# szpiech/garlic

Measured on AMD Instinct MI355X. Metric: LOD-windows/sec (SNPs x inds / winsize), higher is better.
Workload: dtype f64

## Files before the change

garlic_amd/csrc/garlic_hip.hip:

```cpp
#include "../../include/garlic_hip.h"
#include "lod_kernels.hpp"
#include "variant_kernels.hpp"
#include "ld_kernels.hpp"
#include "ld_multi_kernel.hpp"
#include "tgls_ring_kernel.hpp"
#include "tgls_feed_kernel.hpp"
#include "tgls_feed_multi_kernel.hpp"
#include "wlod_strip_kernel.hpp"
#include "wlod_small_kernel.hpp"
#include "coverage_kernel.hpp"
#include "roh_segments_kernel.hpp"
#include "feed_kernel.hpp"
#include "wlod_feed_kernel.hpp"
#include "feed_sort_kernel.hpp"

#include <algorithm>
#include <chrono>
#include <functional>
#include <memory>
#include <mutex>
#include <queue>
#include <cmath>
#include <cstdarg>
#include <cstdio>
// ... 166 lines not shown

struct garlic_panel {
    garlic_ctx *ctx = nullptr;
    int32_t nchr = 0;
    int32_t nind = 0;
    int64_t nloci = 0;
    int64_t nind_pad = 0;
    int64_t nwordrows = 0;
    std::vector<int32_t> chr_nloci;
    std::vector<int64_t> chr_off;
    std::vector<int32_t> pos, cs, ce;
    std::vector<double> gpos, freq;
    bool have_map = false, have_freq = false, have_geno = false, have_gpos = false;
    DevBuf<uint32_t> d_packed;
    DevBuf<int32_t> d_pos, d_cs, d_ce;
    DevBuf<int64_t> d_chr_off;
    DevBuf<double> d_tab;
    bool tab_valid = false;
    double tab_error = 0;
    double tab_min = 0, tabgl_min = 0, glterms_min = 0;
    bool tab_all_finite = false;
    bool seg_valid = false;
    int32_t seg_max_gap = 0;
    std::vector<int64_t> boundaries;
    DevBuf<int32_t> d_blk_counts, d_blk_offsets, d_total;
    DevBuf<int64_t> d_boundaries;
    DevBuf<ChainItem> d_items;
    DevBuf<FeedItem> d_feed_items;
    DevBuf<FillItem> d_fill;
    DevBuf<int32_t> d_counter;
    DevBuf<ChrDev> d_chrs;
    DevBuf<int16_t> d_stage16;
    DevBuf<int64_t> d_row_counts;
    bool have_gl = false;
    std::vector<double> gl_values;
    std::unordered_map<uint64_t, int> gl_code;
    DevBuf<uint8_t> d_codes;
    DevBuf<double> d_tabgl;
    bool tabgl_valid = false;
    DevBuf<double> d_glterms;
    bool glterms_valid = false, glterms_scaled = false;
    int32_t glterms_M = 0;
    double glterms_mu = 0.0;
    int64_t terms_budget = 0;
    DevBuf<double> d_slab[2];
    hipStream_t slab_stream = nullptr;
    hipEvent_t ev_slab_begin = nullptr, ev_slab_built[2] = {}, ev_slab_read[2] = {};
    DevBuf<int32_t> d_slab_queues;
    int32_t last_slab_blocks = 0, last_n_slabs = 0;

    int tabgl_ncodes = 0;
    bool gl_cont = false;
    DevBuf<double> d_glval;
    bool gl_vals_dropped = false;
    bool gl_cover_required = false;
    std::vector<uint8_t> gl_cover;
    DevBuf<double> d_freq;
    bool dfreq_valid = false;
    int gl_terms_by = 0;
    bool have_ld = false, wlod_use_gl = false, rld_valid = false;
    int32_t last_chain_kind = 0;
    int32_t last_feed_form = GARLIC_FEED_FROM_SCORES;
    int64_t last_feed_doubles = 0;
    int32_t ld_winsize = 0;
    struct LdSet {
        int32_t W = 0, group = -1;
        DevBuf<double> skew;
    };
    std::vector<std::unique_ptr<LdSet>> ld_sets;
    int32_t ld_group = -1;
    bool ld_multi_active = false;
    int32_t ld_pair_passes = 0, ld_sum_passes = 0;
    DevBuf<double> d_rld, d_decay, d_stage64;
    DevBuf<uint64_t> d_phase;
    uint64_t geno_epoch = 0;
    CovBits cov_pending{nullptr, nullptr, 0.0};
    bool cov_written = false;
    bool have_phase = false;
    struct {
        DevBuf<uint64_t> sub, m, h, o;
        DevBuf<int32_t> loc, pair, loc_planes;
        DevBuf<double> hf, fwd, bwd, ld;
        DevBuf<LdSumChr> sum_chrs;
        DevBuf<LdPairChr> pair_chrs;
        DevBuf<LdMultiChr> multi_chrs;
        uint64_t planes_key = 0;
        bool planes_valid = false;
        bool fuse_request = false, fused_done = false;
        void release()
        {
            sub.release(); m.release(); h.release(); o.release(); loc.release(); pair.release(); loc_planes.release();
            hf.release(); fwd.release(); bwd.release(); ld.release(); sum_chrs.release(); pair_chrs.release();
            multi_chrs.release();
            planes_valid = false;
        }
    } lds;
    DevBuf<double> d_skew, d_wtab;
    DevBuf<uint8_t> d_valid;
    DevBuf<int2> d_tiles, d_segs;
    DevBuf<WlodStrip> d_strips;
    DevBuf<int32_t> d_feed_blocks;
    std::vector<double> h_tab, h_decay;
    bool wtab_valid = false;
    double wtab_error = 0.0, wtab_mu = 0.0;
    int32_t wtab_M = 0;
    int64_t wtab_rows = 0;
    bool decay_valid = false;
    int32_t decay_M = 0;
    double decay_mu = 0;
    struct ScoreBuf {
        double *p = nullptr;
        size_t cap = 0;
        garlic_ctx *ctx = nullptr;
        int reserve(garlic_ctx *c, size_t n)
        {
            if (n <= cap) return GARLIC_OK;
            release();
            void *q = nullptr;
            int rc = score_alloc(c, n * sizeof(double), &q);
            if (rc) return rc;
            p = (double *)q; cap = n; ctx = c;
            return GARLIC_OK;
        }
        void adopt(garlic_ctx *c, void *q, size_t n) { release(); p = (double *)q; cap = n; ctx = c; }
        void release()
        {
            if (p) (void)score_free(ctx, p);
            p = nullptr; cap = 0;
        }
    } d_out;
    bool placing = false;
    DevBuf<double> d_feed;
    int32_t feed_order = GARLIC_FEED_ORDER_REFERENCE;
    FeedSortScratch fs;
    struct FeedSlot {
        hipStream_t stream = nullptr;
        hipEvent_t ev0 = nullptr, ev1 = nullptr;
        DevBuf<FeedItem> items;
        DevBuf<ChrDev> chrs;
        DevBuf<int32_t> counter;
        DevBuf<int64_t> row_counts;
        DevBuf<double> out, feed;
        FeedSortScratch fs;
    };
    std::vector<FeedSlot *> feed_slots;
    DevBuf<ChainItem> d_multi_items;
    DevBuf<ChrDev> d_multi_chrs, d_multi_gchrs;
    DevBuf<int32_t> d_multi_queues;
    std::vector<int32_t> multi_forms, multi_groups;
    int32_t multi_chain_launches = 0, multi_term_builds = 0;
    garlic_call_stats stats{};
    bool stats_pending = false;
    int stats_slot = 0;
    int64_t n_count_timeouts = 0;
    struct Placement { int32_t drawn = 0, rounds = 0; float best_ms = 0, median_ms = 0, worst_ms = 0, target_ms = 0; int32_t reached = 0; };
    Placement placement;
    struct PlanKey {
        int mode = -1;
        int32_t W = 0, max_gap = 0, ind_begin = 0, ind_count = 0, pitch_align = 0, thin_step = 0;
        uint64_t blocks_hash = 0;
        bool wlod_tuned = false, wlod_strip = false, feed_kernel = false;
        int32_t slab_blocks = 0;
        auto tie() const { return std::tie(mode, W, max_gap, ind_begin, ind_count, pitch_align, thin_step, blocks_hash, wlod_tuned, wlod_strip, feed_kernel, slab_blocks); }
        bool operator==(const PlanKey &o) const { return tie() == o.tie(); }
    };
    struct Plan {
        bool valid = false;
        PlanKey key;
        size_t n_items = 0, n_fill = 0, n_feed_items = 0;
        int feed_per_cu = 1;
        int32_t n_tiles = 0, n_segs = 0, n_strips = 0, n_feed_blocks = 0;
        int64_t n_runs = 0, n_valid = 0;
        struct Slab { int32_t b0, b1; size_t item0, n_items; };
        std::vector<Slab> slabs;
    } plan;
// ... 2229 lines not shown
            if ((rc = p->lds.hf.reserve(p->nloci)) || (rc = p->lds.fwd.reserve(2 * n + 256))) return rc;
            hipLaunchKernelGGL(ld_homfreq_kernel, dim3((unsigned)((p->nloci + 255) / 256)), dim3(256), 0, s, p->lds.loc_planes.p, p->nloci,
                               p->lds.hf.p);
            a_hf = p->lds.hf.p;
            a_c = p->lds.fwd.p;
        }
        if (e == hipSuccess && lds > 48 * 1024) e = hipFuncSetAttribute(fn, hipFuncAttributeMaxDynamicSharedMemorySize, (int)lds);
        if (e != hipSuccess) return fail(GARLIC_ERR_HIP, "LD counts: %s", hipGetErrorString(e));
        const uint64_t *a_m = d_m.p, *a_h = d_h.p;
        const LdPairChr *a_pc = d_pc.p;
        int a_nblk = nblk, a_nchr = p->nchr, a_w = winsize;
        int64_t a_nloci = p->nloci;
        void *kargs[] = {(void *)&a_m, (void *)&a_h, (void *)&a_nblk, (void *)&a_nloci, (void *)&a_pc, (void *)&a_nchr, (void *)&a_w, (void *)&pair,
                         (void *)&a_hf, (void *)&a_c};
        e = hipLaunchKernel(fn, dim3((unsigned)blocks), dim3(256), kargs, lds, s);
        if (e == hipSuccess) e = hipStreamSynchronize(s);
        if (e != hipSuccess) return fail(GARLIC_ERR_HIP, "LD counts: %s", hipGetErrorString(e));
        p->lds.fused_done = fuse_hr2;
    }
    if (pair_lane) {
        std::vector<LdPairChr> pc;
        int64_t blocks = 0;
        for (int c = 0; c < p->nchr; c++) {
            pc.push_back(LdPairChr{p->chr_off[c], p->chr_off[c + 1], blocks});
            blocks += (p->chr_nloci[c] + LD_LANE_T - 1) / LD_LANE_T;
        }
        DevBuf<LdPairChr> &d_pc = p->lds.pair_chrs;
        if ((rc = d_pc.reserve(pc.size()))) return rc;
        e = hipMemcpyAsync(d_pc.p, pc.data(), sizeof(LdPairChr) * pc.size(), hipMemcpyHostToDevice, s);
        const void *fn = lane_dc == 16 ? (phased ? (const void *)ld_pair_lane_kernel<true, 16> : (const void *)ld_pair_lane_kernel<false, 16>)
                                       : (phased ? (const void *)ld_pair_lane_kernel<true, 32> : (const void *)ld_pair_lane_kernel<false, 32>);
        if (e == hipSuccess && lane_lds > 48 * 1024) e = hipFuncSetAttribute(fn, hipFuncAttributeMaxDynamicSharedMemorySize, (int)lane_lds);
        if (e != hipSuccess) return fail(GARLIC_ERR_HIP, "LD counts: %s", hipGetErrorString(e));
        const uint64_t *a_m = d_m.p, *a_h = d_h.p, *a_o = phased ? d_o.p : nullptr, *a_f = phased ? p->d_phase.p : nullptr;
        const LdPairChr *a_pc = d_pc.p;
        int a_nblk = nblk, a_nchr = p->nchr, a_w = winsize, a_stage = lane_stage;
        int64_t a_nloci = p->nloci;
        void *kargs[] = {(void *)&a_m, (void *)&a_h, (void *)&a_o, (void *)&a_f, (void *)&a_nblk, (void *)&a_nloci, (void *)&a_pc,
                         (void *)&a_nchr, (void *)&a_w, (void *)&a_stage, (void *)&pair};
        e = hipLaunchKernel(fn, dim3((unsigned)blocks), dim3(LD_LANE_T), kargs, lane_lds, s);
        if (e == hipSuccess) e = hipStreamSynchronize(s);
        if (e != hipSuccess) return fail(GARLIC_ERR_HIP, "LD counts: %s", hipGetErrorString(e));
    }
    if (pair_flat) {
        const unsigned grid = (unsigned)(((int64_t)p->nloci * winsize + 255) / 256);
        if (phased)
            hipLaunchKernelGGL(ld_pair_flat_kernel<true>, dim3(grid), dim3(256), 0, s, d_m.p, d_h.p, d_o.p, p->d_phase.p, nblk,
                               p->nloci, p->d_chr_off.p, p->nchr, winsize, pair);
        else
            hipLaunchKernelGGL(ld_pair_flat_kernel<false>, dim3(grid), dim3(256), 0, s, d_m.p, d_h.p, (const uint64_t *)nullptr,
                               (const uint64_t *)nullptr, nblk, p->nloci, p->d_chr_off.p, p->nchr, winsize, pair);
    }
    for (int c = 0; !pair_tiled && !pair_flat && !pair_lane && !pair_mfma && c < p->nchr; c++) {
        if (phased)
            hipLaunchKernelGGL(ld_pair_phased_kernel, dim3((unsigned)p->chr_nloci[c]), dim3(256), 0, s, d_m.p,
                               d_h.p, d_o.p, p->d_phase.p, nblk, p->nloci, p->chr_off[c], p->chr_off[c + 1],
                               winsize, pair);
        else
            hipLaunchKernelGGL(ld_pair_kernel, dim3((unsigned)p->chr_nloci[c]), dim3(256), 0, s, d_m.p, d_h.p,
                               nblk, p->nloci, p->chr_off[c], p->chr_off[c + 1], winsize, pair);
    }
    e = hipGetLastError();
    if (e == hipSuccess && where == GARLIC_HOST) {
        e = hipMemcpyAsync(locus_counts, loc, sizeof(int32_t) * p->nloci * 2, hipMemcpyDeviceToHost, s);
        if (e == hipSuccess)
            e = hipMemcpyAsync(pair_counts, pair, sizeof(int32_t) * npair, hipMemcpyDeviceToHost, s);
    }
    if (e == hipSuccess) e = hipStreamSynchronize(s);
    if (e != hipSuccess) return fail(GARLIC_ERR_HIP, "LD counts: %s", hipGetErrorString(e));
    return GARLIC_OK;
}

int garlic_ld_finish(garlic_panel *p, int32_t winsize, int32_t phased, const int32_t *locus_counts,
                     const int32_t *pair_counts, double *ld_out, int32_t where)
{
    int rc;
    if ((rc = ld_check(p, winsize, phased))) return rc;
    if (!locus_counts || !pair_counts) return fail(GARLIC_ERR_INVALID, "count buffers are required");
    hipStream_t s = p->ctx->stream;
    const size_t n = (size_t)p->nloci * winsize;
    DevBuf<int32_t> &d_loc = p->lds.loc, &d_pair = p->lds.pair;
    DevBuf<double> &d_hf = p->lds.hf, &d_fwd = p->lds.fwd, &d_bwd = p->lds.bwd, &d_ld = p->lds.ld;
    DevBuf<LdSumChr> &d_sum_chrs = p->lds.sum_chrs;
    const int32_t *loc = locus_counts, *pair = pair_counts;
    hipError_t e = hipSuccess;
    if (where == GARLIC_HOST) {
        if ((rc = d_loc.reserve((size_t)p->nloci * 2)) || (rc = d_pair.reserve(n * 2))) return rc;
        e = hipMemcpyAsync(d_loc.p, locus_counts, sizeof(int32_t) * p->nloci * 2, hipMemcpyHostToDevice, s);
        if (e == hipSuccess)
            e = hipMemcpyAsync(d_pair.p, pair_counts, sizeof(int32_t) * n * 2, hipMemcpyHostToDevice, s);
        loc = d_loc.p; pair = d_pair.p;
    }
    if (winsize <= LD_SMALL_MAX_W && !getenv("GARLIC_LD_NO_FLAT")) {
        if ((rc = d_hf.reserve(p->nloci))) return rc;
        double *ld = ld_out;
        if (where == GARLIC_HOST || !ld_out) {
            if ((rc = d_ld.reserve(n))) return rc;
            ld = d_ld.p;
        }
        if (e == hipSuccess) e = hipMemsetAsync(ld, 0, sizeof(double) * n, s);
        if (e == hipSuccess && phased) e = hipMemcpyAsync(d_hf.p, p->freq.data(), sizeof(double) * p->nloci, hipMemcpyHostToDevice, s);
        if (e != hipSuccess) return fail(GARLIC_ERR_HIP, "LD finish: %s", hipGetErrorString(e));
        if (!phased)
            hipLaunchKernelGGL(ld_homfreq_kernel, dim3((unsigned)((p->nloci + 255) / 256)), dim3(256), 0, s, loc, p->nloci, d_hf.p);
        garlic_ctx *ctx = p->ctx;
        const int slot = (int)(ctx->n_calls % garlic_ctx::HIST);
        (void)hipEventRecord(ctx->hist0[slot], s);
        hipLaunchKernelGGL(ld_sum_flat_kernel, dim3((unsigned)((n + 255) / 256)), dim3(256), 0, s, pair, d_hf.p, p->d_chr_off.p,
                           p->nchr, p->nloci, winsize, ld);
        (void)hipEventRecord(ctx->hist1[slot], s);
        ctx->n_calls++;
        e = hipGetLastError();
        if (e != hipSuccess) return fail(GARLIC_ERR_HIP, "LD finish: %s", hipGetErrorString(e));
        if ((rc = install_ld(p, winsize, ld, false))) return rc;
        if (where == GARLIC_HOST && ld_out) {
            e = hipMemcpyAsync(ld_out, ld, sizeof(double) * n, hipMemcpyDeviceToHost, s);
            if (e == hipSuccess) e = hipStreamSynchronize(s);
            if (e != hipSuccess) return fail(GARLIC_ERR_HIP, "LD finish: %s", hipGetErrorString(e));
        }
        return GARLIC_OK;
    }
    const int col_threads = (winsize + 16 + WAVE - 1) / WAVE * WAVE;
    const bool by_snp = ld_sums_by_snp(winsize);
    const bool have_table = p->lds.fused_done && by_snp;
    p->lds.fused_done = false;
    const bool tiled = by_snp || (winsize <= LD_SUM_MAX_W && !getenv("GARLIC_LD_SUM_L2"));
    const int sum_b = by_snp ? std::min(LD_COL_B, col_threads - winsize) : LD_SUM_B;
    if ((rc = d_hf.reserve(p->nloci)) || (rc = d_fwd.reserve(by_snp ? 2 * n + 256 : n)) || (!by_snp && (rc = d_bwd.reserve(n))))
        return rc;
    double *ld = ld_out;
    const bool weights_only = by_snp && !ld_out;
    if (!weights_only && (where == GARLIC_HOST || !ld_out)) {
        if ((rc = d_ld.reserve(n))) return rc;
        ld = d_ld.p;
    }
    if (weights_only) {
    } else if (by_snp) {
        for (int c = 0; c < p->nchr && e == hipSuccess; c++) {
            const int64_t lo = p->chr_off[c], hi = p->chr_off[c + 1], from = std::max(lo, hi - winsize + 1);
            if (hi > from) e = hipMemsetAsync(ld + from * winsize, 0, sizeof(double) * (size_t)(hi - from) * winsize, s);
        }
    } else {
        e = hipMemsetAsync(ld, 0, sizeof(double) * n, s);
    }
    if (e != hipSuccess) return fail(GARLIC_ERR_HIP, "LD finish: %s", hipGetErrorString(e));
    if (phased) {
        e = hipMemcpyAsync(d_hf.p, p->freq.data(), sizeof(double) * p->nloci, hipMemcpyHostToDevice, s);
        if (e != hipSuccess) return fail(GARLIC_ERR_HIP, "LD finish: %s", hipGetErrorString(e));
    } else {
        hipLaunchKernelGGL(ld_homfreq_kernel, dim3((unsigned)((p->nloci + 255) / 256)), dim3(256), 0, s, loc,
                           p->nloci, d_hf.p);
    }
    std::vector<LdSumChr> sum_chrs;
    int64_t sum_blocks = 0;
    for (int c = 0; tiled && c < p->nchr; c++) {
        const int64_t nstarts = p->chr_off[c + 1] - p->chr_off[c] - winsize + 1;
        if (nstarts < 1) continue;
        sum_chrs.push_back(LdSumChr{p->chr_off[c], nstarts, sum_blocks});
        sum_blocks += (nstarts + sum_b - 1) / sum_b;
    }
    if (tiled && (rc = d_sum_chrs.reserve(std::max<size_t>(sum_chrs.size(), 1)))) return rc;
    if (by_snp && (rc = reserve_skew(p, winsize, false))) return rc;
    for (int c = 0; c < p->nchr; c++) {
        const int64_t lo = p->chr_off[c], hi = p->chr_off[c + 1];
        const size_t hr2_lds = sizeof(double) * (LD_HR2_T + winsize + (size_t)LD_HR2_T * (winsize + 1));
        if (have_table)
            ;
        else if (by_snp && hr2_lds <= 64 * 1024 && !getenv("GARLIC_LD_HR2_PLAIN"))
            hipLaunchKernelGGL(ld_hr2_tile_kernel, dim3((unsigned)((hi - lo + LD_HR2_T - 1) / LD_HR2_T)), dim3(256),
                               hr2_lds, s, pair, d_hf.p, lo, hi, winsize, d_fwd.p);
        else if (by_snp)
            hipLaunchKernelGGL(ld_hr2_kernel<true>, dim3((unsigned)(hi - lo)), dim3(128), 0, s, pair, d_hf.p, lo, hi,
                               winsize, d_fwd.p, (double *)nullptr);
        else
            hipLaunchKernelGGL(ld_hr2_kernel<false>, dim3((unsigned)(hi - lo)), dim3(256), 0, s, pair, d_hf.p, lo, hi,
                               winsize, d_fwd.p, d_bwd.p);
        if (hi - lo >= winsize && !tiled)
            hipLaunchKernelGGL(ld_sum_kernel, dim3((unsigned)(hi - lo - winsize + 1)), dim3(256), 0, s, d_fwd.p, d_bwd.p,
                               lo, winsize, ld);
    }
    if (tiled && !sum_chrs.empty()) {
        e = hipMemcpyAsync(d_sum_chrs.p, sum_chrs.data(), sizeof(LdSumChr) * sum_chrs.size(), hipMemcpyHostToDevice, s);
        if (e != hipSuccess) return fail(GARLIC_ERR_HIP, "LD finish: %s", hipGetErrorString(e));
        const int threads = by_snp ? col_threads : (winsize + WAVE - 1) / WAVE * WAVE;
        const int col_pieces = (threads * 8 + 1023) / 1024;
        const size_t lds = by_snp ? sizeof(double) * std::max<size_t>((size_t)LD_COL_BATCH * LD_COL_NBATCH * col_pieces * 128 + 130, (size_t)threads * 17)
                                  : sizeof(double) * 2 * (2 * (size_t)winsize - 1 + 128 + threads);
        garlic_ctx *ctx = p->ctx;
        const int slot = (int)(ctx->n_calls % garlic_ctx::HIST);
        (void)hipEventRecord(ctx->hist0[slot], s);
        if (by_snp) {
            static_assert(LD_COL_MAX_THREADS <= 128 * LD_COL_MAX_PIECES, "one instantiation per request count");
            const void *fn = col_pieces == 1 ? (const void *)ld_sum_col_kernel<1> : col_pieces == 2 ? (const void *)ld_sum_col_kernel<2>
                           : col_pieces == 3 ? (const void *)ld_sum_col_kernel<3> : col_pieces == 4 ? (const void *)ld_sum_col_kernel<4>
                                                                                                    : (const void *)ld_sum_col_kernel<5>;
            if (lds > 48 * 1024) {
                e = hipFuncSetAttribute(fn, hipFuncAttributeMaxDynamicSharedMemorySize, (int)lds);
                if (e != hipSuccess) return fail(GARLIC_ERR_HIP, "LD finish: %s", hipGetErrorString(e));
            }
            const double *a_c = d_fwd.p;
            const LdSumChr *a_chrs = d_sum_chrs.p;
            int a_nchr = (int)sum_chrs.size(), a_w = winsize, a_b = sum_b;
            double *a_ld = ld, *a_d = p->d_skew.p + SKEW_FRONT;
            unsigned a_nwork = (unsigned)sum_blocks;
            void *kargs[] = {(void *)&a_c, (void *)&a_chrs, (void *)&a_nchr, (void *)&a_w, (void *)&a_b, (void *)&a_ld, (void *)&a_d, (void *)&a_nwork};
            e = hipLaunchKernel(fn, dim3((a_nwork + 7u) / 8u * 8u), dim3(threads), kargs, lds, s);
            if (e != hipSuccess) return fail(GARLIC_ERR_HIP, "LD finish: %s", hipGetErrorString(e));
        }
        else
            hipLaunchKernelGGL(ld_sum_tiled_kernel, dim3((unsigned)sum_blocks), dim3(threads), lds, s, d_fwd.p, d_bwd.p,
                               d_sum_chrs.p, (int)sum_chrs.size(), winsize, ld);
        (void)hipEventRecord(ctx->hist1[slot], s);
        ctx->n_calls++;
    }
    e = hipGetLastError();
    if (e != hipSuccess) return fail(GARLIC_ERR_HIP, "LD finish: %s", hipGetErrorString(e));
    if ((rc = install_ld(p, winsize, ld, by_snp))) return rc;
    if (where == GARLIC_HOST && ld_out) {
        e = hipMemcpyAsync(ld_out, ld, sizeof(double) * n, hipMemcpyDeviceToHost, s);
        if (e == hipSuccess) e = hipStreamSynchronize(s);
        if (e != hipSuccess) return fail(GARLIC_ERR_HIP, "LD finish: %s", hipGetErrorString(e));
    }
    return GARLIC_OK;
}

int garlic_panel_compute_ld(garlic_panel *p, int32_t winsize, int32_t phased, const int32_t *sub_idx,
                            int32_t n_sub, double *ld_out, int32_t where)
{
    int rc;
    if ((rc = ld_check(p, winsize, phased))) return rc;
    DevBuf<int32_t> &d_loc = p->lds.loc, &d_pair = p->lds.pair;
    const bool fuse = ld_pairs_on_mfma(winsize, phased) && ld_sums_by_snp(winsize) && !getenv("GARLIC_LD_UNFUSED");
    if ((rc = d_loc.reserve((size_t)p->nloci * 2)) || (rc = d_pair.reserve(fuse ? 2 : (size_t)p->nloci * winsize * 2)))
        return rc;
    p->lds.fuse_request = fuse;
    if ((rc = garlic_ld_counts(p, winsize, phased, sub_idx, n_sub, d_loc.p, d_pair.p, GARLIC_DEVICE))) {
        p->lds.fuse_request = false;
        return rc;
    }
    if (where == GARLIC_DEVICE || !ld_out)
        return garlic_ld_finish(p, winsize, phased, d_loc.p, d_pair.p, ld_out, GARLIC_DEVICE);
    DevBuf<double> &d_ld = p->lds.ld;
    if ((rc = d_ld.reserve((size_t)p->nloci * winsize))) return rc;
    rc = garlic_ld_finish(p, winsize, phased, d_loc.p, d_pair.p, d_ld.p, GARLIC_DEVICE);
    if (rc == GARLIC_OK) {
        hipError_t e = hipMemcpy(ld_out, d_ld.p, sizeof(double) * p->nloci * winsize, hipMemcpyDeviceToHost);
        if (e != hipSuccess) rc = fail(GARLIC_ERR_HIP, "LD copy-out: %s", hipGetErrorString(e));
    }
    return rc;
}

static int ld_col_threads(int32_t winsize) { return (winsize + 16 + WAVE - 1) / WAVE * WAVE; }

struct LdMultiPlan {
    std::vector<int32_t> uniq;
    std::vector<std::vector<int32_t>> groups;
    size_t n_shared = 0;
    int32_t wtab = 0;
};
static LdMultiPlan ld_multi_plan(const int32_t *winsizes, int32_t n_sizes)
{
    LdMultiPlan plan;
    plan.uniq.assign(winsizes, winsizes + n_sizes);
    std::sort(plan.uniq.begin(), plan.uniq.end());
    plan.uniq.erase(std::unique(plan.uniq.begin(), plan.uniq.end()), plan.uniq.end());
    const char *solo_env = getenv("GARLIC_LD_MULTI_SOLO");
    const bool solo = solo_env && atoi(solo_env) != 0;
    std::vector<int32_t> sharing, alone;
    for (int32_t w : plan.uniq) (!solo && ld_sums_by_snp(w) ? sharing : alone).push_back(w);
    if (sharing.size() < 2) {
        alone = plan.uniq;
        sharing.clear();
    }
    for (int32_t w : sharing) {
        const bool fits = !plan.groups.empty() && plan.groups.back().size() < (size_t)LDM_MAX_SIZES &&
                          ldms_lds_bytes(ld_col_threads(w), (int)plan.groups.back().size()) <= LDMS_LDS_MAX;
        if (!fits) plan.groups.emplace_back();
        plan.groups.back().push_back(w);
    }
    plan.n_shared = plan.groups.size();
    plan.wtab = sharing.empty() ? 0 : sharing.back();
    for (int32_t w : alone) plan.groups.push_back(std::vector<int32_t>{w});
    return plan;
}

typedef std::vector<std::unique_ptr<garlic_panel::LdSet>> LdSetPool;
static std::unique_ptr<garlic_panel::LdSet> ld_pool_take(LdSetPool &pool, int32_t winsize)
{
    for (size_t i = 0; i < pool.size(); i++)
// ... 1632 lines not shown
```

garlic_amd/csrc/ld_kernels.hpp:

```cpp
#pragma once
#include "lod_kernels.hpp"
#include "tgls_math.hpp"
#include "variant_kernels.hpp"

namespace garlic {

__device__ __forceinline__ double x86_nan_if_nan(double v)
{
    return v != v ? f64_from_bits(X86_DEFAULT_NAN) : v;
}

__device__ __forceinline__ uint32_t ld_writelane(uint32_t v, int lane, uint32_t old)
{
    asm("v_writelane_b32 %0, %1, %2" : "+v"(old) : "s"(v), "n"(lane));
    return old;
}

template <bool PHASED>
__global__ void __launch_bounds__(256)
ld_planes_kernel(const uint32_t *__restrict__ packed, int64_t nwordrows, int nblk,
                 const uint64_t *__restrict__ submask, int64_t nloci, uint64_t *__restrict__ planeM,
                 uint64_t *__restrict__ planeH, uint64_t *__restrict__ planeO, int32_t *__restrict__ counts)
{
    __shared__ int32_t red[4][16][2];
    const int lane = threadIdx.x & 63, wave = threadIdx.x >> 6;
    const int64_t w = blockIdx.x;
    const int64_t l0 = w * 16 - GOFF;
    int32_t hom = 0, tot = 0;
    for (int blk0 = wave; blk0 < nblk; blk0 += 32) {
        uint32_t words[8];
#pragma unroll
        for (int u = 0; u < 8; u++)
            words[u] = packed[((int64_t)min(blk0 + 4 * u, nblk - 1) * nwordrows + w) * WAVE + lane];
#pragma unroll
        for (int u = 0; u < 8; u++) {
            const int blk = blk0 + 4 * u;
            if (blk >= nblk) break;
            const uint32_t word = words[u];
            const uint64_t sub = submask[blk];
            uint32_t mlo = 0, mhi = 0, hlo = 0, hhi = 0, olo = 0, ohi = 0, tlo = 0, thi = 0;
#pragma unroll
            for (int q = 0; q < 16; q++) {
                const uint32_t code = (word >> (2 * q)) & 3u;
                const uint64_t m = __ballot(code != 3u);
                const uint64_t h = __ballot(code == 0u || code == 2u);
                mlo = ld_writelane((uint32_t)m, q, mlo);
                mhi = ld_writelane((uint32_t)(m >> 32), q, mhi);
                hlo = ld_writelane((uint32_t)h, q, hlo);
                hhi = ld_writelane((uint32_t)(h >> 32), q, hhi);
                if (PHASED) {
                    const uint64_t two = __ballot(code == 2u), one = __ballot(code == 1u);
                    tlo = ld_writelane((uint32_t)two, q, tlo);
                    thi = ld_writelane((uint32_t)(two >> 32), q, thi);
                    olo = ld_writelane((uint32_t)one, q, olo);
                    ohi = ld_writelane((uint32_t)(one >> 32), q, ohi);
                }
            }
            if (lane < 16) {
                const uint64_t m = ((uint64_t)mhi << 32) | mlo, h = ((uint64_t)hhi << 32) | hlo;
                hom += __popcll(h);
                tot += __popcll(m);
                const int64_t l = l0 + lane;
                if (l >= 0 && l < nloci) {
                    planeM[(int64_t)blk * nloci + l] = m & sub;
                    if (!PHASED) planeH[(int64_t)blk * nloci + l] = h & sub;
                    if (PHASED) {
                        planeH[(int64_t)blk * nloci + l] = (((uint64_t)thi << 32) | tlo) & sub;
                        planeO[(int64_t)blk * nloci + l] = (((uint64_t)ohi << 32) | olo) & sub;
                    }
                }
            }
        }
    }
    if (lane < 16) { red[wave][lane][0] = hom; red[wave][lane][1] = tot; }
    __syncthreads();
    if (threadIdx.x < 16) {
        const int64_t l = l0 + threadIdx.x;
        if (l >= 0 && l < nloci) {
            counts[2 * l + 0] = red[0][threadIdx.x][0] + red[1][threadIdx.x][0] + red[2][threadIdx.x][0] + red[3][threadIdx.x][0];
            counts[2 * l + 1] = red[0][threadIdx.x][1] + red[1][threadIdx.x][1] + red[2][threadIdx.x][1] + red[3][threadIdx.x][1];
        }
    }
}

__global__ void __launch_bounds__(256)
ld_pair_kernel(const uint64_t *__restrict__ planeM, const uint64_t *__restrict__ planeH, int nblk,
// ... 359 lines not shown
        ld[s * W + k] = x86_nan_if_nan(acc);
    }
}

constexpr int LD_SUM_B = 32;
constexpr int LD_SUM_AHEAD = 4;
constexpr int LD_SUM_MAX_W = 256;
struct LdSumChr {
    int64_t lo;
    int64_t nstarts;
    int64_t block0;
};
__global__ void __launch_bounds__(LD_SUM_MAX_W)
ld_sum_tiled_kernel(const double *__restrict__ fwd, const double *__restrict__ bwd,
                    const LdSumChr *__restrict__ chrs, int nchr, int W, double *__restrict__ ld)
{
    extern __shared__ double ld_rows[];
    const int k = threadIdx.x, nthreads = blockDim.x, RW = 2 * W - 1, L = RW + 128 + nthreads;
    int c = 0;
    while (c + 1 < nchr && (int64_t)blockIdx.x >= chrs[c + 1].block0) c++;
    const int64_t s0 = chrs[c].lo + ((int64_t)blockIdx.x - chrs[c].block0) * LD_SUM_B;
    const int ns = (int)min<int64_t>(LD_SUM_B, chrs[c].lo + chrs[c].nstarts - s0);
    const int nsteps = ns + W - 1;
    auto term = [&](int64_t i, int x) -> double {
        return x < W - 1 ? bwd[i * W + (W - 1 - x)] : (x == W - 1 ? 1.0 : fwd[i * W + (x - W + 1)]);
    };
    double acc[LD_SUM_B];
#pragma unroll
    for (int q = 0; q < LD_SUM_B; q++) acc[q] = 0.0;
    const int x0 = min(k, RW - 1), x1 = min(k + nthreads, RW - 1);
    double pre[LD_SUM_AHEAD][2];
#pragma unroll
    for (int u = 0; u < LD_SUM_AHEAD; u++) {
        const int64_t i = s0 + min(u, nsteps - 1);
        pre[u][0] = term(i, x0);
        pre[u][1] = term(i, x1);
    }
    for (int j0 = 0; j0 < nsteps; j0 += LD_SUM_AHEAD) {
#pragma unroll
        for (int u = 0; u < LD_SUM_AHEAD; u++) {
            const int j = j0 + u;
            if (j >= nsteps) break;
            double *row = ld_rows + (j & 1) * L + 64;
            if (k < RW) row[k] = pre[u][0];
            if (k + nthreads < RW) row[k + nthreads] = pre[u][1];
            {
                const int64_t i = s0 + min(j + LD_SUM_AHEAD, nsteps - 1);
                pre[u][0] = term(i, x0);
                pre[u][1] = term(i, x1);
            }
            __syncthreads();
            const int qlo = max(0, j - W + 1), qhi = min(j, ns - 1);
            const double *cp = row + (W - 1 + k - j);
#pragma unroll
            for (int g = 0; g < LD_SUM_B; g += 16) {
                if (g > qhi || g + 15 < qlo) continue;
                double t[16];
#pragma unroll
                for (int r = 0; r < 16; r++) t[r] = cp[g + r];
#pragma unroll
                for (int r = 0; r < 16; r++)
                    if (g + r >= qlo && g + r <= qhi) {
                        acc[g + r] += t[r];
                        asm volatile("" ::: "memory");
                    }
            }
        }
    }
    if (k < W) {
#pragma unroll
        for (int q = 0; q < LD_SUM_B; q++)
            if (q < ns) ld[(s0 + q) * W + k] = x86_nan_if_nan(acc[q]);
    }
}

constexpr int LD_COL_B = 32;
constexpr int LD_COL_MAX_THREADS = 576;
#ifndef GARLIC_LD_COL_BATCH
#define GARLIC_LD_COL_BATCH 4
#endif
constexpr int LD_COL_BATCH = GARLIC_LD_COL_BATCH;
constexpr int LD_COL_NBATCH = 4;
constexpr int LD_COL_MAX_PIECES = 5;

__device__ __forceinline__ void ld_col_wait(int n)
{
    switch (n) {
#define LD_COL_WAIT_CASE(k) case k: asm volatile("s_waitcnt vmcnt(" #k ")" ::: "memory"); break;
        LD_COL_WAIT_CASE(0)
        LD_COL_WAIT_CASE(1)
        LD_COL_WAIT_CASE(2)
        LD_COL_WAIT_CASE(3)
        LD_COL_WAIT_CASE(4)
        LD_COL_WAIT_CASE(5)
        LD_COL_WAIT_CASE(6)
        LD_COL_WAIT_CASE(7)
        LD_COL_WAIT_CASE(8)
        LD_COL_WAIT_CASE(9)
        LD_COL_WAIT_CASE(10)
        LD_COL_WAIT_CASE(11)
        LD_COL_WAIT_CASE(12)
        LD_COL_WAIT_CASE(13)
        LD_COL_WAIT_CASE(14)
        LD_COL_WAIT_CASE(15)
        LD_COL_WAIT_CASE(16)
        LD_COL_WAIT_CASE(17)
        LD_COL_WAIT_CASE(18)
        LD_COL_WAIT_CASE(19)
        LD_COL_WAIT_CASE(20)
        LD_COL_WAIT_CASE(21)
        LD_COL_WAIT_CASE(22)
        LD_COL_WAIT_CASE(23)
        LD_COL_WAIT_CASE(24)
        LD_COL_WAIT_CASE(25)
        LD_COL_WAIT_CASE(26)
        LD_COL_WAIT_CASE(27)
        LD_COL_WAIT_CASE(28)
        LD_COL_WAIT_CASE(29)
        LD_COL_WAIT_CASE(30)
        LD_COL_WAIT_CASE(31)
        LD_COL_WAIT_CASE(32)
        LD_COL_WAIT_CASE(33)
        LD_COL_WAIT_CASE(34)
        LD_COL_WAIT_CASE(35)
        LD_COL_WAIT_CASE(36)
        LD_COL_WAIT_CASE(37)
        LD_COL_WAIT_CASE(38)
        LD_COL_WAIT_CASE(39)
        LD_COL_WAIT_CASE(40)
        LD_COL_WAIT_CASE(41)
        LD_COL_WAIT_CASE(42)
        LD_COL_WAIT_CASE(43)
        LD_COL_WAIT_CASE(44)
        LD_COL_WAIT_CASE(45)
        LD_COL_WAIT_CASE(46)
        LD_COL_WAIT_CASE(47)
        LD_COL_WAIT_CASE(48)
        LD_COL_WAIT_CASE(49)
        LD_COL_WAIT_CASE(50)
        LD_COL_WAIT_CASE(51)
        LD_COL_WAIT_CASE(52)
        LD_COL_WAIT_CASE(53)
        LD_COL_WAIT_CASE(54)
        LD_COL_WAIT_CASE(55)
        LD_COL_WAIT_CASE(56)
        LD_COL_WAIT_CASE(57)
        LD_COL_WAIT_CASE(58)
        LD_COL_WAIT_CASE(59)
        LD_COL_WAIT_CASE(60)
        LD_COL_WAIT_CASE(61)
        LD_COL_WAIT_CASE(62)
        LD_COL_WAIT_CASE(63)
#undef LD_COL_WAIT_CASE
    default: asm volatile("s_waitcnt vmcnt(0)" ::: "memory"); break;
    }
}

#define LD_COL_ADD(q) "v_add_f64 %[a" #q "], %[a" #q "], %[h]\n\t"
#define LD_COL_OPS(a)                                                                                              \
    [a0] "+v"(a[0]), [a1] "+v"(a[1]), [a2] "+v"(a[2]), [a3] "+v"(a[3]), [a4] "+v"(a[4]), [a5] "+v"(a[5]),          \
    [a6] "+v"(a[6]), [a7] "+v"(a[7]), [a8] "+v"(a[8]), [a9] "+v"(a[9]), [a10] "+v"(a[10]), [a11] "+v"(a[11]),      \
    [a12] "+v"(a[12]), [a13] "+v"(a[13]), [a14] "+v"(a[14]), [a15] "+v"(a[15]), [a16] "+v"(a[16]),                 \
    [a17] "+v"(a[17]), [a18] "+v"(a[18]), [a19] "+v"(a[19]), [a20] "+v"(a[20]), [a21] "+v"(a[21]),                 \
    [a22] "+v"(a[22]), [a23] "+v"(a[23]), [a24] "+v"(a[24]), [a25] "+v"(a[25]), [a26] "+v"(a[26]),                 \
    [a27] "+v"(a[27]), [a28] "+v"(a[28]), [a29] "+v"(a[29]), [a30] "+v"(a[30]), [a31] "+v"(a[31])
#define LD_COL_JUMP "s_getpc_b64 s[98:99]\n\ts_add_u32 s98, s98, %[off]\n\ts_addc_u32 s99, s99, 0\n\ts_setpc_b64 s[98:99]\n\t"
__device__ __forceinline__ void ld_col_adds(double (&a)[LD_COL_B], double h, bool ascending, int first)
{
    static_assert(LD_COL_B == 32, "32 adds are written out");
    const uint32_t off = (uint32_t)__builtin_amdgcn_readfirstlane(first * 8 + (ascending ? 12 + 32 * 8 + 4 : 12));
    asm volatile(LD_COL_JUMP
                 LD_COL_ADD(31) LD_COL_ADD(30) LD_COL_ADD(29) LD_COL_ADD(28) LD_COL_ADD(27) LD_COL_ADD(26)
                 LD_COL_ADD(25) LD_COL_ADD(24) LD_COL_ADD(23) LD_COL_ADD(22) LD_COL_ADD(21) LD_COL_ADD(20)
                 LD_COL_ADD(19) LD_COL_ADD(18) LD_COL_ADD(17) LD_COL_ADD(16) LD_COL_ADD(15) LD_COL_ADD(14)
                 LD_COL_ADD(13) LD_COL_ADD(12) LD_COL_ADD(11) LD_COL_ADD(10) LD_COL_ADD(9) LD_COL_ADD(8) LD_COL_ADD(7)
                 LD_COL_ADD(6) LD_COL_ADD(5) LD_COL_ADD(4) LD_COL_ADD(3) LD_COL_ADD(2) LD_COL_ADD(1) LD_COL_ADD(0)
                 "s_branch LD_COL_END_%=\n\t"
                 LD_COL_ADD(0) LD_COL_ADD(1) LD_COL_ADD(2) LD_COL_ADD(3) LD_COL_ADD(4) LD_COL_ADD(5)
                 LD_COL_ADD(6) LD_COL_ADD(7) LD_COL_ADD(8) LD_COL_ADD(9) LD_COL_ADD(10) LD_COL_ADD(11) LD_COL_ADD(12)
                 LD_COL_ADD(13) LD_COL_ADD(14) LD_COL_ADD(15) LD_COL_ADD(16) LD_COL_ADD(17) LD_COL_ADD(18)
                 LD_COL_ADD(19) LD_COL_ADD(20) LD_COL_ADD(21) LD_COL_ADD(22) LD_COL_ADD(23) LD_COL_ADD(24)
                 LD_COL_ADD(25) LD_COL_ADD(26) LD_COL_ADD(27) LD_COL_ADD(28) LD_COL_ADD(29) LD_COL_ADD(30)
                 LD_COL_ADD(31)
                 "LD_COL_END_%=:\n\t"
                 : LD_COL_OPS(a) : [h] "v"(h), [off] "s"(off) : "s98", "s99", "scc");
}
template <int PIECES>
__global__ void __launch_bounds__(LD_COL_MAX_THREADS)
ld_sum_col_kernel(const double *__restrict__ C, const LdSumChr *__restrict__ chrs, int nchr, int W, int B,
                  double *__restrict__ ld, double *__restrict__ D, unsigned nwork)
{
    const unsigned per_xcd = gridDim.x >> 3;
    const unsigned vblock = (blockIdx.x & 7u) * per_xcd + (blockIdx.x >> 3);
    if (vblock >= nwork) return;
    constexpr int BATCH = LD_COL_BATCH, NB = LD_COL_NBATCH, NRING = BATCH * NB, STEADY = (NB - 2) * BATCH * PIECES;
    static_assert(STEADY <= 63, "requests that can be counted");
    extern __shared__ double ld_rows[];
    const int tl = threadIdx.x, P = 2 * W;
    const int wave = __builtin_amdgcn_readfirstlane(threadIdx.x >> 6);
    int c = 0;
    while (c + 1 < nchr && (int64_t)vblock >= chrs[c + 1].block0) c++;
    const int64_t s0 = chrs[c].lo + ((int64_t)vblock - chrs[c].block0) * B;
    const int ns = (int)min<int64_t>(B, chrs[c].lo + chrs[c].nstarts - s0);
    const int nsteps = ns + W - 1, nbatches = (nsteps + BATCH - 1) / BATCH;
    const uint32_t ring = (uint32_t)(uintptr_t)(__attribute__((address_space(3))) double *)ld_rows;
    constexpr uint32_t row_bytes = (uint32_t)PIECES * 1024u, ring_bytes = row_bytes * NRING;
    const uint32_t lane16 = (uint32_t)(tl & 63) * 16u;
    const char *req_row = reinterpret_cast<const char *>(C + s0 * P);
    int req_e = W - 1, req_left = nsteps;
    uint32_t req_off = 0;
    auto request_batch = [&]() {
#pragma unroll
        for (int u = 0; u < BATCH; u++) {
            if (req_left > 0) {
                const char *g = req_row + (int64_t)(req_e & ~1) * 8;
#pragma unroll
                for (int q = 0; q < PIECES; q++)
                    asm volatile("s_mov_b32 m0, %0\n\ts_nop 0\n\tglobal_load_lds_dwordx4 %1, %2"
                                 :: "s"(ring + req_off + (uint32_t)q * 1024u), "v"(lane16), "s"(g + q * 1024) : "memory");
                req_row += (int64_t)P * 8;
                req_e--;
                req_left--;
            }
            req_off += row_bytes;
        }
        if (req_off == ring_bytes) req_off = 0;
    };
    if (wave == 0)
        for (int k = 0; k < NB - 1; k++) request_batch();
    double acc[LD_COL_B];
#pragma unroll
    for (int q = 0; q < LD_COL_B; q++) acc[q] = 0.0;
    uint32_t rd_addr = ring + (uint32_t)tl * 8u;
    const uint32_t rd_end = rd_addr + ring_bytes;
    uint32_t odd = (uint32_t)(W - 1) & 1u;
    static_assert(BATCH % 2 == 0, "the parity of W-1-j repeats per batch");
    for (int k = 0; k < nbatches; k++) {
        if (wave == 0) {
            const int rows_later = min(nsteps, (k + NB - 1) * BATCH) - (k + 1) * BATCH;
            if (rows_later == (NB - 2) * BATCH) asm volatile("s_waitcnt vmcnt(%0)" ::"n"(STEADY) : "memory");
            else ld_col_wait(max(rows_later, 0) * PIECES);
        }
        __syncthreads();
        if (wave == 0) request_batch();
        const int j0 = k * BATCH;
        double h[BATCH];
#pragma unroll
        for (int u = 0; u < BATCH; u++)
            asm volatile("ds_read_b64 %0, %1" : "=v"(h[u]) : "v"(rd_addr + (uint32_t)u * row_bytes + ((odd ^ (uint32_t)(u & 1)) * 8u)) : "memory");
        asm volatile("s_waitcnt lgkmcnt(0)" ::: "memory");
        rd_addr += BATCH * row_bytes;
        if (rd_addr == rd_end) rd_addr -= ring_bytes;
#pragma unroll
        for (int u = 0; u < BATCH; u++) {
            const int j = j0 + u;
#ifdef GARLIC_LDS_ABL_NO_ADDS
            if (j < nsteps && h[u] == 1.2345e-300) {
#else
            if (j < nsteps) {
#endif
                const bool leaving = j >= W;
                ld_col_adds(acc, h[u], leaving,
                            leaving ? j - W + 1 : (j < LD_COL_B - 1 ? LD_COL_B - 1 - j : 0));
            }
        }
    }
#ifndef GARLIC_LDS_ABL_NO_LD
    if (ld) {
#pragma unroll
        for (int q = 0; q < LD_COL_B; q++) {
            const int k = tl - q;
            if (q < ns && k >= 0 && k < W) ld[(s0 + q) * W + k] = x86_nan_if_nan(acc[q]);
        }
    }
#else
    if (acc[0] == 1.2345e-300) ld[s0 * W + tl] = acc[1] + acc[2] + acc[3] + acc[31] + acc[16];
#endif
#ifdef GARLIC_LDS_ABL_NO_D
    if (acc[5] != 1.2345e-300) return;
#endif
    if (!D) return;
    __syncthreads();
    double *tile = ld_rows;
    const int nthreads = blockDim.x;
    for (int q0 = 0; q0 < LD_COL_B; q0 += 16) {
#pragma unroll
        for (int u = 0; u < 16; u++)
            if (q0 == 0) tile[tl * 17 + u] = reciprocal_x86(x86_nan_if_nan(acc[u]));
            else tile[tl * 17 + u] = reciprocal_x86(x86_nan_if_nan(acc[16 + u]));
        __syncthreads();
        for (int e = tl; e < nthreads * 16; e += nthreads) {
            const int t2 = e >> 4, u = e & 15, q = q0 + u, k = t2 - q;
            if (q < ns && k >= 0 && k < W) D[(s0 + t2) * W + k] = tile[t2 * 17 + u];
        }
        __syncthreads();
    }
}

}

namespace garlic {

constexpr int LDM_TI = 128;
typedef int ldm_i32x4 __attribute__((ext_vector_type(4)));

typedef int ldm_i32x8 __attribute__((ext_vector_type(8)));
typedef float ldm_f32x16 __attribute__((ext_vector_type(16)));

__device__ __forceinline__ uint32_t ldm_spread8(uint32_t x)
{
    uint32_t t = (x | (x << 12)) & 0x000F000Fu;
    t = (t | (t << 6)) & 0x03030303u;
    return (t | (t << 3)) & 0x11111111u;
}

constexpr int LDM_XT = 33;
constexpr size_t LDM_XT_BYTES = ((size_t)4 * 32 * LDM_XT + 256) * 8;

template <int NJ, bool HR2>
__global__ void __launch_bounds__(256, 2)
ld_pair_mfma_kernel(const uint64_t *__restrict__ planeM, const uint64_t *__restrict__ planeH, int nblk, int64_t nloci,
                    const LdPairChr *__restrict__ chrs, int nchr, int W, int32_t *__restrict__ pair,
                    const double *__restrict__ hf, double *__restrict__ C)
{
    constexpr int NT = 4 + NJ - 1;
    static_assert(NT * 32 <= 256, "one staged SNP per thread");
    constexpr int BUF = 2 * NT * WAVE * 16;
// ... 132 lines not shown
```

Measured before the change: 7.169 billion.

## Order LD column-sum blocks into chains with predecessor start gating

Remaps block IDs so that each XCD runs several chains of adjacent work blocks. The chain count is derived from occupancy, B and W. Each block waits, with a bounded spin, until its predecessor in the chain has signalled that it passed a set batch, which keeps neighbouring blocks that read overlapping rows of C close in time so they share L2. This adds an epoch-stamped device flag buffer, an occupancy query, and spin-wait latency that can stall blocks if the estimate of resident blocks is wrong.

After: 7.251 billion, median of 3. No clear change (+1.1%).

```diff
diff --git a/garlic_amd/csrc/garlic_hip.hip b/garlic_amd/csrc/garlic_hip.hip
--- a/garlic_amd/csrc/garlic_hip.hip
+++ b/garlic_amd/csrc/garlic_hip.hip
@@ -272,6 +272,9 @@
         DevBuf<int32_t> loc, pair, loc_planes;
         DevBuf<double> hf, fwd, bwd, ld;
         DevBuf<LdSumChr> sum_chrs;
+        DevBuf<unsigned> sum_started;
+        unsigned sum_epoch = 0;
+        int sum_occ_w = 0, sum_occ = 0;
         DevBuf<LdPairChr> pair_chrs;
         DevBuf<LdMultiChr> multi_chrs;
         uint64_t planes_key = 0;
@@ -281,6 +284,7 @@
         {
             sub.release(); m.release(); h.release(); o.release(); loc.release(); pair.release(); loc_planes.release();
             hf.release(); fwd.release(); bwd.release(); ld.release(); sum_chrs.release(); pair_chrs.release();
+            sum_started.release();
             multi_chrs.release();
             planes_valid = false;
         }
@@ -2676,6 +2680,7 @@
     DevBuf<int32_t> &d_loc = p->lds.loc, &d_pair = p->lds.pair;
     DevBuf<double> &d_hf = p->lds.hf, &d_fwd = p->lds.fwd, &d_bwd = p->lds.bwd, &d_ld = p->lds.ld;
     DevBuf<LdSumChr> &d_sum_chrs = p->lds.sum_chrs;
+    DevBuf<unsigned> &d_started = p->lds.sum_started;
     const int32_t *loc = locus_counts, *pair = pair_counts;
     hipError_t e = hipSuccess;
     if (where == GARLIC_HOST) {
@@ -2797,8 +2802,29 @@
             int a_nchr = (int)sum_chrs.size(), a_w = winsize, a_b = sum_b;
             double *a_ld = ld, *a_d = p->d_skew.p + SKEW_FRONT;
             unsigned a_nwork = (unsigned)sum_blocks;
-            void *kargs[] = {(void *)&a_c, (void *)&a_chrs, (void *)&a_nchr, (void *)&a_w, (void *)&a_b, (void *)&a_ld, (void *)&a_d, (void *)&a_nwork};
-            e = hipLaunchKernel(fn, dim3((a_nwork + 7u) / 8u * 8u), dim3(threads), kargs, lds, s);
+            const unsigned grid = (a_nwork + LD_ORDER_XCDS - 1) / LD_ORDER_XCDS * LD_ORDER_XCDS;
+            if (p->lds.sum_occ_w != winsize) {
+                int per_cu = 0;
+                e = hipOccupancyMaxActiveBlocksPerMultiprocessor(&per_cu, fn, threads, lds);
+                if (e != hipSuccess) return fail(GARLIC_ERR_HIP, "LD finish: %s", hipGetErrorString(e));
+                p->lds.sum_occ = std::max(1, per_cu);
+                p->lds.sum_occ_w = winsize;
+            }
+            const unsigned resident = (unsigned)p->lds.sum_occ * (unsigned)std::max(1, ctx->n_cu / (int)LD_ORDER_XCDS);
+            unsigned a_chains = ld_order_chains(resident, (unsigned)sum_b, (unsigned)winsize, LD_COL_EXTRA_STEPS);
+            if (const char *env = getenv("GARLIC_LD_SUM_CHAINS")) a_chains = (unsigned)std::max(1, atoi(env));
+            if (d_started.cap < grid) {
+                if ((rc = d_started.reserve(grid))) return rc;
+                e = hipMemsetAsync(d_started.p, 0, sizeof(unsigned) * d_started.cap, s);
+                if (e != hipSuccess) return fail(GARLIC_ERR_HIP, "LD finish: %s", hipGetErrorString(e));
+                p->lds.sum_epoch = 0;
+            }
+            unsigned *a_started = d_started.p;
+            unsigned a_epoch = ++p->lds.sum_epoch;
+            if (a_epoch == 0) a_epoch = p->lds.sum_epoch = 1;
+            void *kargs[] = {(void *)&a_c, (void *)&a_chrs, (void *)&a_nchr, (void *)&a_w, (void *)&a_b, (void *)&a_ld, (void *)&a_d, (void *)&a_nwork,
+                             (void *)&a_chains, (void *)&a_started, (void *)&a_epoch};
+            e = hipLaunchKernel(fn, dim3(grid), dim3(threads), kargs, lds, s);
             if (e != hipSuccess) return fail(GARLIC_ERR_HIP, "LD finish: %s", hipGetErrorString(e));
         }
         else
diff --git a/garlic_amd/csrc/ld_kernels.hpp b/garlic_amd/csrc/ld_kernels.hpp
--- a/garlic_amd/csrc/ld_kernels.hpp
+++ b/garlic_amd/csrc/ld_kernels.hpp
@@ -2,6 +2,7 @@
 #include "lod_kernels.hpp"
 #include "tgls_math.hpp"
 #include "variant_kernels.hpp"
+#include "ld_sum_order.hpp"
 
 namespace garlic {
 
@@ -527,6 +528,8 @@
 constexpr int LD_COL_BATCH = GARLIC_LD_COL_BATCH;
 constexpr int LD_COL_NBATCH = 4;
 constexpr int LD_COL_MAX_PIECES = 5;
+constexpr unsigned LD_COL_EXTRA_STEPS = 12;
+constexpr uint64_t LD_COL_WAIT_TICKS = 2000;
 
 __device__ __forceinline__ void ld_col_wait(int n)
 {
@@ -633,10 +636,10 @@
 template <int PIECES>
 __global__ void __launch_bounds__(LD_COL_MAX_THREADS)
 ld_sum_col_kernel(const double *__restrict__ C, const LdSumChr *__restrict__ chrs, int nchr, int W, int B,
-                  double *__restrict__ ld, double *__restrict__ D, unsigned nwork)
-{
-    const unsigned per_xcd = gridDim.x >> 3;
-    const unsigned vblock = (blockIdx.x & 7u) * per_xcd + (blockIdx.x >> 3);
+                  double *__restrict__ ld, double *__restrict__ D, unsigned nwork, unsigned n_chains,
+                  unsigned *__restrict__ started, unsigned epoch)
+{
+    const unsigned vblock = ld_order_group(blockIdx.x, gridDim.x / LD_ORDER_XCDS, n_chains);
     if (vblock >= nwork) return;
     constexpr int BATCH = LD_COL_BATCH, NB = LD_COL_NBATCH, NRING = BATCH * NB, STEADY = (NB - 2) * BATCH * PIECES;
     static_assert(STEADY <= 63, "requests that can be counted");
@@ -671,8 +674,17 @@
         }
         if (req_off == ring_bytes) req_off = 0;
     };
-    if (wave == 0)
+    const int k_started = (B + BATCH - 1) / BATCH;
+    if (wave == 0) {
         for (int k = 0; k < NB - 1; k++) request_batch();
+        const unsigned pred = ld_order_predecessor(blockIdx.x, n_chains);
+        if (pred != blockIdx.x) {
+            const uint64_t give_up = wall_clock64() + LD_COL_WAIT_TICKS;
+            while (__hip_atomic_load(started + pred, __ATOMIC_RELAXED, __HIP_MEMORY_SCOPE_AGENT) != epoch &&
+                   wall_clock64() < give_up)
+                __builtin_amdgcn_s_sleep(8);
+        }
+    }
     double acc[LD_COL_B];
 #pragma unroll
     for (int q = 0; q < LD_COL_B; q++) acc[q] = 0.0;
@@ -688,6 +700,7 @@
         }
         __syncthreads();
         if (wave == 0) request_batch();
+        if (k == k_started && tl == WAVE) __hip_atomic_store(started + blockIdx.x, epoch, __ATOMIC_RELAXED, __HIP_MEMORY_SCOPE_AGENT);
         const int j0 = k * BATCH;
         double h[BATCH];
 #pragma unroll
diff --git a/garlic_amd/csrc/ld_sum_order.hpp b/garlic_amd/csrc/ld_sum_order.hpp
--- /dev/null
+++ b/garlic_amd/csrc/ld_sum_order.hpp
@@ -0,0 +1,33 @@
+#pragma once
+
+#if defined(__HIPCC__)
+#define GARLIC_LD_ORDER_HD __host__ __device__ __forceinline__
+#else
+#define GARLIC_LD_ORDER_HD inline
+#endif
+
+namespace garlic {
+
+constexpr unsigned LD_ORDER_XCDS = 8;
+
+GARLIC_LD_ORDER_HD unsigned ld_order_chains(unsigned resident, unsigned B, unsigned W, unsigned extra)
+{
+    const unsigned life = B + W - 1 + extra;
+    const unsigned n = (unsigned)(((unsigned long long)resident * B + life / 2) / life);
+    return n < 1u ? 1u : n;
+}
+
+GARLIC_LD_ORDER_HD unsigned ld_order_group(unsigned id, unsigned per_xcd, unsigned n_chains)
+{
+    const unsigned xcd = id % LD_ORDER_XCDS, x = id / LD_ORDER_XCDS;
+    const unsigned chain = x % n_chains, pos = x / n_chains;
+    const unsigned len = per_xcd / n_chains, longer = per_xcd % n_chains;
+    return xcd * per_xcd + chain * len + (chain < longer ? chain : longer) + pos;
+}
+
+GARLIC_LD_ORDER_HD unsigned ld_order_predecessor(unsigned id, unsigned n_chains)
+{
+    return id / LD_ORDER_XCDS >= n_chains ? id - LD_ORDER_XCDS * n_chains : id;
+}
+
+}
```
